# M-Igashi/mp3rgain

Measured on AMD Instinct MI355X. Metric: stereo PCM samples/s through IIR+RMS+histogram, higher is better.
Workload: dtype f64

## Files before the change

mp3rgain_amd/csrc/rg_capi.hip:

```cpp
#include <atomic>
#include <chrono>
#include <hip/hip_runtime.h>

#include <dlfcn.h>
#include <math.h>
#include <stdarg.h>
#include <stdio.h>
#include <string.h>

#include <string>
#include <vector>

#include "rg_ctx.h"

extern "C" {
hipError_t rg_launch_k1_halo(const RgTrackDev *, uint32_t, uint32_t, const RgCoefDev *, uint32_t *,
                             unsigned long long *, unsigned long long *, hipStream_t);
hipError_t rg_launch_track_results(const uint32_t *, const unsigned long long *, const RgTrackDev *,
                                   const unsigned long long *, rg_track_result *, uint32_t, hipStream_t);
hipError_t rg_launch_album_merge(const uint32_t *, const unsigned long long *, uint32_t, uint32_t *, double *,
                                 hipStream_t);
hipError_t rg_launch_album_result(const uint32_t *, const double *, rg_album_result *, hipStream_t);
hipError_t rg_launch_album_reduce_gathered(const uint32_t *, uint32_t, uint32_t *, double *, hipStream_t);
hipError_t rg_launch_peak_all(const void *, uint64_t, uint32_t, unsigned long long *, hipStream_t);
hipError_t rg_launch_synth_fill(float *, uint64_t, uint32_t, uint32_t, uint64_t, uint64_t, hipStream_t);
}

namespace {
thread_local std::string g_create_error;
}

int rg_set_err(rg_ctx *c, int code, const char *fmt, ...) {
    char buf[512];
    va_list ap;
    va_start(ap, fmt);
    vsnprintf(buf, sizeof buf, fmt, ap);
    va_end(ap);
    if (c) c->err = buf; else g_create_error = buf;
    return code;
}

int rg_rate_index(uint32_t sr) {
    for (int i = 0; i < RG_NUM_RATES; ++i)
        if (RG_RATE_TABLE[i].sample_rate == sr) return i;
    return -1;
}

int rg_bind_device(rg_ctx *c) {
    RG_HIP(c, hipSetDevice(c->device));
    return RG_OK;
}

namespace {

int32_t round_to_i32(double v) {
    double r = round(v);
    if (r != r) return 0;
    if (r >= 2147483647.0) return INT32_MAX;
    if (r <= -2147483648.0) return INT32_MIN;
    return (int32_t)r;
}

int drain_timing(rg_ctx *c) {
    for (int k = 0; k < RG_MAX_SLOTS; ++k) {
        RgSlot &S = c->slots[k];
        for (size_t i = 0; i < S.ev_used; ++i) {
            float ms = 0.f;
            RG_HIP(c, hipEventElapsedTime(&ms, S.ev_pool[i].first, S.ev_pool[i].second));
            c->timing_sum_ms += ms;
            c->timing_count += 1;
// ... 151 lines not shown
        else S.stream = c->slots[k % RG_SLOT_STREAMS].stream;
        if (e == hipSuccess) e = hipEventCreateWithFlags(&S.staging_done, hipEventDisableTiming);
        if (e == hipSuccess) e = hipEventCreateWithFlags(&S.batch_done, hipEventDisableTiming);
        if (e == hipSuccess) e = hipEventCreateWithFlags(&S.album_done, hipEventDisableTiming);
        if (e == hipSuccess) e = S.d_album_hist.reserve(RG_HISTOGRAM_SIZE + 2);
        if (e == hipSuccess) S.d_album_peak.p = reinterpret_cast<double *>(S.d_album_hist.p + RG_HISTOGRAM_SIZE);
        if (e == hipSuccess) e = S.d_album_result.reserve(1);
        if (e == hipSuccess) e = S.h_album_result.reserve(1);
    }
    if (e != hipSuccess) {
        rg_set_err(nullptr, RG_ERR_DEVICE, "stream / buffer creation: %s", hipGetErrorString(e));
        rg_destroy(c);
        return nullptr;
    }

    std::vector<RgCoefDev> coefs(RG_NUM_RATES);
    for (int i = 0; i < RG_NUM_RATES; ++i) {
        rg_design_rate(RG_RATE_TABLE[i], &c->design[i]);
        memcpy(coefs[i].ya, RG_RATE_TABLE[i].yule_a, sizeof coefs[i].ya);
        memcpy(coefs[i].yb, RG_RATE_TABLE[i].yule_b, sizeof coefs[i].yb);
        memcpy(coefs[i].ba, RG_RATE_TABLE[i].butter_a, sizeof coefs[i].ba);
        memcpy(coefs[i].bb, RG_RATE_TABLE[i].butter_b, sizeof coefs[i].bb);
    }
    if ((e = c->d_coefs.reserve(RG_NUM_RATES)) != hipSuccess ||
        (e = hipMemcpy(c->d_coefs.p, coefs.data(), sizeof(RgCoefDev) * RG_NUM_RATES, hipMemcpyHostToDevice)) !=
            hipSuccess) {
        rg_set_err(nullptr, RG_ERR_DEVICE, "context allocation: %s", hipGetErrorString(e));
        rg_destroy(c);
        return nullptr;
    }
    check_hw_queues(c);
    return c;
}

extern "C" void rg_destroy(rg_ctx *c) {
    if (!c) return;
    (void)hipSetDevice(c->device);
    (void)sync_all(c);
    (void)rg_comm_destroy(c);
    for (int k = 0; k < RG_MAX_SLOTS; ++k) {
        RgSlot &S = c->slots[k];
        for (auto &p : S.ev_pool) {
            (void)hipEventDestroy(p.first);
            (void)hipEventDestroy(p.second);
        }
        S.d_desc.release();
        S.h_desc.release();
        S.d_tm_rec.release();
        S.d_tm_win.release();
        S.d_hist.release();
        S.d_nonfinite.release();
        S.d_imprecise.release();
        S.d_k1_bad.release();
        S.d_results.release();
        S.h_results.release();
        S.d_album_hist.release();
        S.d_album_peak.p = nullptr;
        S.d_album_result.release();
        S.d_gather.release();
        S.h_album_result.release();
        if (S.staging_done) (void)hipEventDestroy(S.staging_done);
        if (S.batch_done) (void)hipEventDestroy(S.batch_done);
        if (S.album_done) (void)hipEventDestroy(S.album_done);
        if (S.stream && k < RG_SLOT_STREAMS) (void)hipStreamDestroy(S.stream);
    }
    if (c->user_ev) (void)hipEventDestroy(c->user_ev);
    c->d_coefs.release();
    c->d_peak_bits.release();
    c->d_arena.release();
    c->d_wav.release();
    c->d_flac_blob.release();
    c->d_flac_work.release();
    c->h_flac_stage.release();
    c->d_flac_md5.release();
    c->d_mp3_crc.release();
    c->d_rip.release();
    c->d_stats.release();
    c->d_spectrum.release();
    c->d_dr.release();
    c->d_stereo.release();
    c->d_clicks.release();
    c->d_flacenc.release();
    c->d_flacenc_out.release();
    c->d_flacenc_verify.release();
    c->d_ancestry.release();
    c->d_fprint.release();
    c->d_fp_codes.release();
    c->d_tempo.release();
    c->d_tp_onsets.release();
    c->d_key.release();
    c->d_key_decim.release();
    c->d_key_rows.release();
    c->d_rs.release();
    c->d_rs_y.release();
    c->h_mp3_crc.release();
    if (c->file_pool && c->file_pool_free) c->file_pool_free(c->file_pool);
    c->file_pool = nullptr;
    c->d_mp3_tab.release();
    c->d_mp3_is.release();
    c->d_mp3_units.release();
    c->d_mp3_tracks.release();
    c->d_mp3_huff.release();
    c->d_mp3_recs.release();
    c->d_mp3_main.release();
    if (c->mp3_pipe && c->mp3_pipe_free) c->mp3_pipe_free(c->mp3_pipe);
    c->mp3_pipe = nullptr;
// ... 716 lines not shown
```

mp3rgain_amd/csrc/rg_ctx.h:

```cpp
#pragma once

#include <hip/hip_runtime.h>

#include <map>
#include <string>
#include <vector>

#include "rg_design.h"
#include "rg_device.h"
#include "rg_tm.h"

template <typename T>
struct DevBuf {
    T *p = nullptr;
    size_t cap = 0;
    hipError_t reserve(size_t n) {
        if (n <= cap) return hipSuccess;
        if (p) (void)hipFree(p);
        p = nullptr;
        cap = 0;
        size_t want = n + n / 4 + 16;
        hipError_t e = hipMalloc((void **)&p, want * sizeof(T));
        if (e == hipSuccess) cap = want;
        return e;
// ... 5 lines not shown
    }
};

template <typename T>
struct PinnedBuf {
    T *p = nullptr;
    size_t cap = 0;
    hipError_t reserve(size_t n) {
        if (n <= cap) return hipSuccess;
        if (p) (void)hipHostFree(p);
        p = nullptr;
        cap = 0;
        size_t want = n + n / 4 + 16;
        hipError_t e = hipHostMalloc((void **)&p, want * sizeof(T), hipHostMallocDefault);
        if (e == hipSuccess) cap = want;
        return e;
    }
    void release() {
        if (p) (void)hipHostFree(p);
        p = nullptr;
        cap = 0;
    }
};

struct RgTmDeviceTables {
    RgTmDesign design;
    double *d_blob = nullptr;
    RgTmGeom geom{};
    RgTmFixTables fix{};
};

enum { RG_TUNE_TM_SEGMENT = 1, RG_TUNE_TM_TARGET_LANES = 2, RG_TUNE_PIPELINE_SLOTS = 3, RG_TUNE_TM_WINDOWS = 4, RG_TUNE_INGEST_CHUNK_KIB = 5,
       RG_TUNE_GPU_MP3_DECODE = 6, RG_TUNE_LOADER_THREADS = 7, RG_TUNE_ALBUM_PARTS = 10, RG_TUNE_PARTS_MIN_BPU = 11,
       RG_TUNE_STAGE_BYTES = 12, RG_TUNE_GROUP_BYTES = 13, RG_TUNE_GPU_FLAC_DECODE = 14 };

#define RG_MAX_SLOTS 8
#define RG_SLOT_STREAMS 4
#define RG_DEFAULT_SLOTS 8

struct RgSlot {
    hipStream_t stream = nullptr;
    hipEvent_t staging_done = nullptr;
    hipEvent_t batch_done = nullptr;
    hipEvent_t album_done = nullptr;
    bool album_pending = false;
    bool staging_pending = false;
    DevBuf<unsigned char> d_desc;
    PinnedBuf<unsigned char> h_desc;
    std::vector<unsigned char> desc_shadow;
    DevBuf<double> d_tm_rec;
    DevBuf<double> d_tm_win;
    DevBuf<uint32_t> d_hist;
    DevBuf<unsigned long long> d_k1_bad;
    DevBuf<uint32_t> d_imprecise;
    DevBuf<uint32_t> d_nonfinite;
    unsigned long long *peak_ptr = nullptr;
    DevBuf<rg_track_result> d_results;
    PinnedBuf<rg_track_result> h_results;
    DevBuf<uint32_t> d_album_hist;
    DevBuf<double> d_album_peak;
    DevBuf<rg_album_result> d_album_result;
    DevBuf<uint32_t> d_gather;
    PinnedBuf<rg_album_result> h_album_result;
    size_t n_enqueued = 0;
    int enq_album = 0;
    const void *enq_base = nullptr;
    size_t enq_bytes = 0;
    bool album_ready = false;
    std::vector<std::pair<hipEvent_t, hipEvent_t>> ev_pool;
    size_t ev_used = 0;
};

struct rg_ctx {
    int device = -1;
    std::string err;
    int kernel_variant = 0;
    uint32_t tune_tm_segment = 0;
    uint32_t tune_tm_windows = 0;
    uint64_t tune_tm_target_lanes = 0;
    int n_slots = RG_DEFAULT_SLOTS;

    RgSlot slots[RG_MAX_SLOTS];
    int cur = 0;
    hipStream_t user_stream = nullptr;
    bool user_attached = false;
    hipEvent_t user_ev = nullptr;
    bool user_dirty = false;
    RgSlot &slot() { return slots[cur]; }
    hipStream_t album_stream() { return user_attached ? user_stream : slots[cur].stream; }
    hipStream_t file_stream() { return album_stream(); }

    RgRateDesign design[RG_NUM_RATES];
    DevBuf<RgCoefDev> d_coefs;
    std::map<uint32_t, RgTmDeviceTables *> tm_tables;

    std::map<uint64_t, std::pair<uint32_t, uint32_t>> tm_choice;

    std::vector<RgTrackDev> h_tracks, h_k1_tracks;
    std::vector<RgTmTrack> h_tm_tracks;

    DevBuf<unsigned long long> d_peak_bits;
    DevBuf<unsigned char> d_mp3_tab;
    DevBuf<int16_t> d_mp3_is;
    DevBuf<unsigned char> d_mp3_units;
    DevBuf<unsigned char> d_mp3_tracks;
    DevBuf<unsigned char> d_mp3_huff;
    DevBuf<unsigned char> d_mp3_recs;
    DevBuf<unsigned char> d_mp3_main;
    bool mp3_tab_ready = false;
    DevBuf<unsigned char> d_mp3_stage[2];
    hipStream_t mp3_copy_stream = nullptr;
    hipEvent_t mp3_set_free[2] = {nullptr, nullptr};
    bool mp3_set_used[2] = {false, false};
    DevBuf<uint32_t> d_mp3_results;
    DevBuf<uint32_t> d_mp3_tiles;
    DevBuf<unsigned char> d_mp3_recs_set[2];
    DevBuf<uint32_t> d_mp3_tiles_set[2];
    DevBuf<uint32_t> d_mp3_perm_set[2];
    DevBuf<uint32_t> d_mp3_sortw_set[2];
    PinnedBuf<uint32_t> h_mp3_results;
    hipEvent_t enqueue_wait_ev = nullptr;
    hipStream_t enqueue_stream = nullptr;
    PinnedBuf<uint32_t> h_mp3_part_counts;
    PinnedBuf<rg_track_result> h_part_results;
    hipEvent_t *mp3_bench_ev = nullptr;
    void *mp3_pipe = nullptr;
    void (*mp3_pipe_free)(void *) = nullptr;
    void *file_pool = nullptr;
    std::vector<std::string> file_errors;
    void (*file_pool_free)(void *) = nullptr;
    int gpu_mp3_decode = 3;
    int gpu_flac_decode = 1;
    DevBuf<unsigned char> d_flac_blob;
    DevBuf<unsigned char> d_flac_work;
    PinnedBuf<unsigned char> h_flac_stage;
    DevBuf<unsigned char> d_flac_md5;
    DevBuf<unsigned char> d_mp3_crc;
    PinnedBuf<unsigned char> h_mp3_crc;
    DevBuf<unsigned char> d_rip;
    DevBuf<unsigned char> d_stats;
    DevBuf<unsigned char> d_spectrum;
    DevBuf<unsigned char> d_dr;
    DevBuf<unsigned char> d_stereo;
    DevBuf<unsigned char> d_clicks;
    DevBuf<unsigned char> d_flacenc;
    DevBuf<unsigned char> d_flacenc_out;
// ... 90 lines not shown
```

mp3rgain_amd/csrc/rg_device.h:

```cpp
#pragma once

#include <stdint.h>

#include "../../include/mp3rgain_amd.h"
#include "../../include/rg_coeffs.h"

#define RG_MAX_TAPS 11

struct RgCoefDev {
    double ya[11];
    double yb[11];
    double ba[3];
    double bb[3];
};

struct RgTrackDev {
    const void *ch0;
    const void *ch1;
    uint64_t frames;
    uint32_t window;
    uint32_t n_windows;
    uint32_t seg_windows;
    uint32_t n_segments;
    uint32_t halo;
    uint32_t coef_idx;
    uint32_t format;
    uint32_t item_base;
    uint32_t sample_rate;
    uint32_t file_type;
    uint32_t track_index;
    uint32_t pad_;
};

#define RG_ONE_MINUS_PERCENTILE (1.0 - 0.95)
```

mp3rgain_amd/csrc/rg_enqueue.hip:

```cpp
#include <stdlib.h>
#include <string.h>

#include <math.h>

#include <algorithm>

#include "rg_ctx.h"

extern "C" {
hipError_t rg_launch_k1_halo(const RgTrackDev *, uint32_t, uint32_t, const RgCoefDev *, uint32_t *,
                             unsigned long long *, unsigned long long *, hipStream_t);
hipError_t rg_launch_track_results(const uint32_t *, const unsigned long long *, const RgTrackDev *,
                                   const unsigned long long *, rg_track_result *, uint32_t, hipStream_t);
hipError_t rg_launch_album_merge(const uint32_t *, const unsigned long long *, uint32_t, uint32_t *, double *,
                                 hipStream_t);
hipError_t rg_launch_tm_main(int fmt, int nch, const RgTmCoef *, const RgTmGeom *, const RgTmTrack *, uint32_t, uint32_t,
                             double *, uint32_t, double *, uint32_t, uint32_t *, uint32_t *, uint64_t, hipStream_t);
hipError_t rg_launch_tm_fix(int nch, const RgTmGeom *, const RgTmFixTables *, const RgTmTrack *, uint32_t, uint32_t,
                            const double *, uint32_t, const double *, uint32_t, uint32_t *, uint32_t *, uint32_t *,
                            unsigned long long *, uint32_t *, rg_track_result *, hipStream_t);
}

namespace {

const uint32_t kMinSegment = 96;

struct TmGroup {
    int rate_idx, fmt, nch;
    std::vector<uint32_t> ids;
    uint64_t frames = 0;
};

int validate(rg_ctx *c, const rg_track_desc *tracks, size_t n, size_t pcm_bytes) {
    for (size_t t = 0; t < n; ++t) {
        const rg_track_desc &d = tracks[t];
        if (rg_rate_index(d.sample_rate) < 0)
            return rg_set_err(c, RG_ERR_UNSUPPORTED_RATE,
                              "Unsupported sample rate: %u Hz. Supported rates: 96000, 88200, 64000, 48000, 44100, "
                              "32000, 24000, 22050, 16000, 12000, 11025, 8000",
                              d.sample_rate);
        if (d.channels == 0) return rg_set_err(c, RG_ERR_INVALID_ARG, "track %zu: channels == 0", t);
        if (d.format > RG_FMT_S32_PLANAR) return rg_set_err(c, RG_ERR_INVALID_ARG, "track %zu: unknown format %u", t, d.format);
        const size_t bps = rg_bytes_per_sample(d.format);
        if (d.offset_bytes % bps) return rg_set_err(c, RG_ERR_INVALID_ARG, "track %zu: offset not sample-aligned", t);
        const uint64_t need = d.offset_bytes + (uint64_t)d.channels * d.frames * bps;
        if (need > pcm_bytes)
            return rg_set_err(c, RG_ERR_INVALID_ARG, "track %zu: extends past the PCM arena (%llu > %zu)", t,
                              (unsigned long long)need, pcm_bytes);
        const uint32_t W = rg_window_samples(d.sample_rate);
        if ((d.frames + W - 1) / W > 0x7FFFFFFFull) return rg_set_err(c, RG_ERR_INVALID_ARG, "track %zu: too long", t);
    }
    return RG_OK;
}

void fill_common(rg_ctx *c, const rg_track_desc &d, const unsigned char *d_base, uint32_t track_index, RgTrackDev &o) {
    const int ri = rg_rate_index(d.sample_rate);
    const size_t bps = rg_bytes_per_sample(d.format);
    memset(&o, 0, sizeof o);
    o.ch0 = d_base + d.offset_bytes;
    o.ch1 = d.channels >= 2 ? d_base + d.offset_bytes + d.frames * bps : nullptr;
    o.frames = d.frames;
    o.window = rg_window_samples(d.sample_rate);
    o.n_windows = (uint32_t)((d.frames + o.window - 1) / o.window);
    o.coef_idx = (uint32_t)ri;
    o.format = d.format;
    o.sample_rate = d.sample_rate;
    o.file_type = RG_FILE_MP3;
    o.track_index = track_index;
    (void)c;
}

int finish_k1_list(rg_ctx *c, RgTrackDev *list, size_t n, uint32_t *total_items) {
    uint64_t total_windows = 0;
    for (size_t t = 0; t < n; ++t) total_windows += list[t].n_windows;
    uint32_t seg_windows = 1;
    if (total_windows > (1u << 18)) {
        uint64_t s = total_windows >> 17;
        seg_windows = (uint32_t)(s > 16 ? 16 : s);
    }
    uint64_t items = 0;
    for (size_t t = 0; t < n; ++t) {
        RgTrackDev &o = list[t];
        if (t > 0 && list[t - 1].coef_idx != o.coef_idx) items = (items + 63) & ~(uint64_t)63;
        if (c->design[o.coef_idx].stable) {
            o.seg_windows = seg_windows;
            o.halo = c->design[o.coef_idx].halo_frames;
        } else {
            o.seg_windows = o.n_windows ? o.n_windows : 1;
            o.halo = 0xFFFFFFFFu;
        }
        o.n_segments = (o.n_windows + o.seg_windows - 1) / o.seg_windows;
        o.item_base = (uint32_t)items;
        items += o.n_segments;
        if (items > 0x7FFFFFFFull) return rg_set_err(c, RG_ERR_INVALID_ARG, "batch too large");
    }
    *total_items = (uint32_t)items;
    return RG_OK;
}

int get_tm_tables(rg_ctx *c, int rate_idx, uint32_t L, RgTmDeviceTables **out, uint32_t m = 1) {
    const uint32_t key = ((uint32_t)rate_idx << 24) | (m << 16) | L;
    auto it = c->tm_tables.find(key);
    if (it != c->tm_tables.end()) {
        *out = it->second;
        return it->second->design.ok ? RG_OK : RG_ERR_INVALID_ARG;
    }
    RgTmDeviceTables *tb = new RgTmDeviceTables();
    rg_tm_design(RG_RATE_TABLE[rate_idx], L, &tb->design, m);
    c->tm_tables[key] = tb;
    *out = tb;
    const RgTmDesign &D = tb->design;
    if (!D.ok) return RG_ERR_INVALID_ARG;
    const size_t nT = D.T.size(), nG = D.Gp.size(), nY = D.PhiY.size(), nB = D.PhiB.size();
    const size_t nL = (size_t)D.H10 * 12 + (size_t)(D.L - D.H10) * 2;
    const size_t nST = D.ST.size();
    const size_t total = nT + nG + nY + nB + 24 + 12 + 100 + 12 + 8 + nL + 2 + nST;
    std::vector<double> blob(total, 0.0);
    size_t o = 0;
    const size_t oT = o; memcpy(&blob[o], D.T.data(), nT * 8); o += nT;
    const size_t oG = o; memcpy(&blob[o], D.Gp.data(), nG * 8); o += nG;
    const size_t oY = o; if (nY) memcpy(&blob[o], D.PhiY.data(), nY * 8); o += nY;
    const size_t oB = o; if (nB) memcpy(&blob[o], D.PhiB.data(), nB * 8); o += nB;
    const size_t oX = o; memcpy(&blob[o], &D.Xs[0][0], 24 * 8); o += 24;
    const size_t oS = o; memcpy(&blob[o], D.sigma0, 12 * 8); o += 12;
    memcpy(&blob[o], D.Wf, 100 * 8); o += 100;
    if (nST) memcpy(&blob[o], &D.ST[(size_t)(D.L - 1) * 12], 12 * 8);
    o += 12;
    o = (o + 1) & ~(size_t)1;
    const size_t oL = o;
    for (uint32_t n = 0; n < D.H10; ++n)
        for (int j = 0; j < 12; ++j) blob[o++] = D.T[(size_t)n * 12 + j];
    for (uint32_t n = D.H10; n < D.L; ++n) { blob[o++] = D.T[(size_t)n * 12 + 10]; blob[o++] = D.T[(size_t)n * 12 + 11]; }
    o = (o + 1) & ~(size_t)1;
    const size_t oST = o;
    if (nST) memcpy(&blob[o], D.ST.data(), nST * 8);
    o += nST;
    RG_HIP(c, hipMalloc((void **)&tb->d_blob, total * 8));
    RG_HIP(c, hipMemcpy(tb->d_blob, blob.data(), total * 8, hipMemcpyHostToDevice));
    RgTmGeom &g = tb->geom;
    g.L = D.L;
    g.W = D.W;
    g.k = D.W / D.L;
    g.H10 = D.H10;
    g.rounds = D.rounds;
    g.rounds_fast = D.rounds_fast;
    g.warm = 1u << D.rounds;
    g.fix_windows = (RG_TM_BLOCK - g.warm) / g.k;
    g.block = rg_tm_choose_block(D.L, D.H10, m);
    g.m = m;
// ... 173 lines not shown
    if (S.album_pending) {
        RG_HIP(c, hipStreamWaitEvent(s, S.album_done, 0));
        S.album_pending = false;
    }

    if (S.staging_pending) {
        RG_HIP(c, hipEventSynchronize(S.staging_done));
        S.staging_pending = false;
    }

    c->h_tracks.resize(n ? n : 1);
    c->h_k1_tracks.resize(n ? n : 1);
    c->h_tm_tracks.resize(n ? n : 1);
    const size_t acc_words = n * (size_t)(RG_HISTOGRAM_SIZE + 3);
    RG_HIP(c, S.d_hist.reserve(acc_words));
    S.peak_ptr = reinterpret_cast<unsigned long long *>(S.d_hist.p + n * (size_t)RG_HISTOGRAM_SIZE);
    uint32_t *const done_ptr = S.d_hist.p + n * (size_t)(RG_HISTOGRAM_SIZE + 2);
    RG_HIP(c, S.d_results.reserve(n));
    RG_HIP(c, S.h_results.reserve(n));
    if (n > S.d_nonfinite.cap) {
        RG_HIP(c, S.d_nonfinite.reserve(n));
        RG_HIP(c, hipMemsetAsync(S.d_nonfinite.p, 0, S.d_nonfinite.cap * sizeof(uint32_t), s));
    }
    if (n > S.d_imprecise.cap) {
        RG_HIP(c, S.d_imprecise.reserve(n));
        RG_HIP(c, hipMemsetAsync(S.d_imprecise.p, 0, S.d_imprecise.cap * sizeof(uint32_t), s));
    }

    const unsigned char *base = (const unsigned char *)d_pcm_base;
    const bool use_tm = c->kernel_variant != 1;

    std::vector<TmGroup> groups;
    size_t n_k1 = 0;
    for (size_t t = 0; t < n; ++t) {
        fill_common(c, tracks[t], base, (uint32_t)t, c->h_tracks[t]);
        const int ri = rg_rate_index(tracks[t].sample_rate);
        const bool tm_rate = !(c->force_exact.size() == n && c->force_exact[t]);
        if (use_tm && tm_rate && c->design[ri].stable) {
            const int nch = tracks[t].channels >= 2 ? 2 : 1;
            TmGroup *g = nullptr;
            for (auto &q : groups)
                if (q.rate_idx == ri && q.fmt == (int)tracks[t].format && q.nch == nch) { g = &q; break; }
            if (!g) {
                groups.push_back(TmGroup{ri, (int)tracks[t].format, nch, {}, 0});
                g = &groups.back();
            }
            g->ids.push_back((uint32_t)t);
            g->frames += tracks[t].frames;
        } else {
            c->h_k1_tracks[n_k1++] = c->h_tracks[t];
        }
    }
    uint32_t k1_items = 0;
    rc = finish_k1_list(c, c->h_k1_tracks.data(), n_k1, &k1_items);
    if (rc != RG_OK) return rc;

    struct GroupLaunch {
        RgTmDeviceTables *tb;
        RgTmCoef K;
        size_t list_off, list_n;
        uint32_t main_grid, fix_grid, total_recs, total_windows;
        int fmt, nch;
    };
    std::vector<GroupLaunch> launches;
    size_t tm_off = 0;
    size_t max_rec_doubles = 0, max_win_doubles = 0;
    for (const TmGroup &g : groups) {
        GroupLaunch gl{};
        rc = choose_tm_tables(c, g, tracks, &gl.tb);
        if (rc != RG_OK) return rc;
        const RgTmGeom &geo = gl.tb->geom;
        const rg_rate_coeffs &rcf = RG_RATE_TABLE[g.rate_idx];
        const double scale = g.fmt == RG_FMT_F32_PLANAR ? 32768.0 : (g.fmt == RG_FMT_S16_PLANAR ? 1.0 : 32768.0 / 2147483648.0);
        const RgTmDesign &des = gl.tb->design;
        for (int i = 0; i < 11; ++i) {
            gl.K.b[i] = (des.servo ? (double)((long double)des.g * (long double)rcf.yule_b[i]) : rcf.yule_b[i]) * scale;
            gl.K.a[i] = rcf.yule_a[i];
        }
        for (int i = 0; i < 3; ++i) { gl.K.bb[i] = rcf.butter_b[i]; gl.K.ba[i] = rcf.butter_a[i]; }
        gl.K.c0 = 1e-10;
        gl.K.alpha = des.alpha;
        gl.K.beta = des.beta;
        gl.K.aff_lin = geo.aff_lin;
        gl.K.aff_n = geo.aff_n;
        gl.fmt = g.fmt;
        gl.nch = g.nch;
        gl.list_off = tm_off;
        gl.list_n = g.ids.size();
        uint64_t recs = 0, mb = 0, fb = 0, wins = 0;
        const uint64_t seg_stride = (uint64_t)geo.L * geo.m;
        const uint32_t NB = geo.fix_windows * geo.k;
        const uint32_t geom_block = geo.block;
        for (uint32_t id : g.ids) {
            const RgTrackDev &cd = c->h_tracks[id];
            RgTmTrack &o = c->h_tm_tracks[tm_off++];
            o.ch0 = cd.ch0;
            o.ch1 = cd.ch1;
            o.frames = cd.frames;
            o.nseg = (uint32_t)((cd.frames + seg_stride - 1) / seg_stride);
            o.n_windows = cd.n_windows;
            o.rec_base = (uint32_t)recs;
            o.lane_base = (uint32_t)mb;
            o.fix_block_base = (uint32_t)fb;
            o.track_index = id;
            o.fix_blocks = (o.nseg + NB - 1) / NB;
            o.sample_rate = cd.sample_rate;
            o.file_type = cd.file_type;
// ... 27 lines not shown
    S.enq_base = d_pcm_base;
    S.enq_bytes = pcm_bytes;
    S.album_ready = false;
    const RgTrackDev *d_tracks = nullptr, *d_k1_tracks = nullptr;
    const RgTmTrack *d_tm_tracks = nullptr;
    if (n) {
        const size_t o_all = 0;
        const size_t o_k1 = (o_all + n * sizeof(RgTrackDev) + 15) & ~(size_t)15;
        const size_t o_tm = (o_k1 + n_k1 * sizeof(RgTrackDev) + 15) & ~(size_t)15;
        const size_t blob_bytes = o_tm + tm_off * sizeof(RgTmTrack);
        const size_t old_desc_cap = S.d_desc.cap;
        RG_HIP(c, S.d_desc.reserve(blob_bytes));
        RG_HIP(c, S.h_desc.reserve(blob_bytes));
        if (S.d_desc.cap != old_desc_cap) S.desc_shadow.clear();
        std::vector<unsigned char> blob(blob_bytes, 0);
        memcpy(&blob[o_all], c->h_tracks.data(), n * sizeof(RgTrackDev));
        if (n_k1) memcpy(&blob[o_k1], c->h_k1_tracks.data(), n_k1 * sizeof(RgTrackDev));
        if (tm_off) memcpy(&blob[o_tm], c->h_tm_tracks.data(), tm_off * sizeof(RgTmTrack));
        if (blob != S.desc_shadow) {
            memcpy(S.h_desc.p, blob.data(), blob_bytes);
            RG_HIP(c, hipMemcpyAsync(S.d_desc.p, S.h_desc.p, blob_bytes, hipMemcpyHostToDevice, s));
            RG_HIP(c, hipEventRecord(S.staging_done, s));
            S.staging_pending = true;
            S.desc_shadow.swap(blob);
        }
        d_tracks = reinterpret_cast<const RgTrackDev *>(S.d_desc.p + o_all);
        (void)d_tracks;
        d_k1_tracks = reinterpret_cast<const RgTrackDev *>(S.d_desc.p + o_k1);
        d_tm_tracks = reinterpret_cast<const RgTmTrack *>(S.d_desc.p + o_tm);
        bool cleared = false;
        bool any_main = false;
        for (const GroupLaunch &gl : launches) any_main = any_main || gl.main_grid != 0;
        if (!any_main) {
            RG_HIP(c, hipMemsetAsync(S.d_hist.p, 0, acc_words * sizeof(uint32_t), s));
            cleared = true;
        }

        for (const GroupLaunch &gl : launches) {
            hipEvent_t e1;
            rc = timing_begin(c, &e1);
            if (rc != RG_OK) return rc;
            RG_HIP(c, rg_launch_tm_main(gl.fmt, gl.nch, &gl.K, &gl.tb->geom, d_tm_tracks + gl.list_off,
                                        (uint32_t)gl.list_n, gl.main_grid, S.d_tm_rec.p, gl.total_recs, S.d_tm_win.p,
                                        gl.total_windows, S.d_nonfinite.p, cleared ? nullptr : S.d_hist.p, (uint64_t)acc_words, s));
            if (gl.main_grid != 0) cleared = true;
            if (e1) RG_HIP(c, hipEventRecord(e1, s));
            RG_HIP(c, rg_launch_tm_fix(gl.nch, &gl.tb->geom, &gl.tb->fix, d_tm_tracks + gl.list_off,
                                       (uint32_t)gl.list_n, gl.fix_grid, S.d_tm_rec.p, gl.total_recs, S.d_tm_win.p,
                                       gl.total_windows, S.d_nonfinite.p, S.d_imprecise.p, S.d_hist.p, S.peak_ptr, done_ptr, S.d_results.p, s));
        }
        if (n_k1) {
            RG_HIP(c, S.d_k1_bad.reserve(n));
            RG_HIP(c, hipMemsetAsync(S.d_k1_bad.p, 0xFF, n * sizeof(unsigned long long), s));
            hipEvent_t e1;
            rc = timing_begin(c, &e1);
            if (rc != RG_OK) return rc;
            RG_HIP(c, rg_launch_k1_halo(d_k1_tracks, (uint32_t)n_k1, k1_items, c->d_coefs.p, S.d_hist.p,
                                        S.peak_ptr, S.d_k1_bad.p, s));
            if (e1) RG_HIP(c, hipEventRecord(e1, s));
        }
        RG_HIP(c, rg_launch_track_results(S.d_hist.p, S.peak_ptr, d_k1_tracks, S.d_k1_bad.p, S.d_results.p, (uint32_t)n_k1, s));
    }
    if (album) {
        RG_HIP(c, rg_launch_album_merge(S.d_hist.p, S.peak_ptr, (uint32_t)n, S.d_album_hist.p,
                                        S.d_album_peak.p, s));
        S.album_ready = true;
        if (c->user_attached) {
            RG_HIP(c, hipEventRecord(S.batch_done, s));
            RG_HIP(c, hipStreamWaitEvent(c->user_stream, S.batch_done, 0));
        }
    }
    return RG_OK;
}
```

mp3rgain_amd/csrc/rg_k1_halo.hip:

```cpp
#include <hip/hip_runtime.h>
#include <limits.h>

#include <type_traits>

#include "rg_device.h"
#include "rg_device_inl.h"

#define RG_K1_ELEVEN(f)                                                                                       \
    do {                                                                                                      \
        f(std::integral_constant<int, 0>{}); f(std::integral_constant<int, 1>{}); f(std::integral_constant<int, 2>{});   \
        f(std::integral_constant<int, 3>{});                                                                             \
        __builtin_amdgcn_sched_barrier(0);       \
        f(std::integral_constant<int, 4>{}); f(std::integral_constant<int, 5>{}); f(std::integral_constant<int, 6>{});   \
        f(std::integral_constant<int, 7>{});                                                                             \
        __builtin_amdgcn_sched_barrier(0);                                                                              \
        f(std::integral_constant<int, 8>{}); f(std::integral_constant<int, 9>{}); f(std::integral_constant<int, 10>{}); \
    } while (0)

#define RG_K1_TWELVE(f)                                                                                       \
    do {                                                                                                      \
        f(std::integral_constant<int, 0>{}); f(std::integral_constant<int, 1>{}); f(std::integral_constant<int, 2>{});   \
        f(std::integral_constant<int, 3>{});                                                                             \
        __builtin_amdgcn_sched_barrier(0);                                                                              \
        f(std::integral_constant<int, 4>{}); f(std::integral_constant<int, 5>{}); f(std::integral_constant<int, 6>{});   \
// ... 21 lines not shown
    for (int i = 10; i >= 1; --i) { f.yx[i] = f.yx[i - 1]; f.yy[i] = f.yy[i - 1]; }
    f.yx[0] = s;
    double acc = 0.0;
#pragma unroll
    for (int i = 1; i < 11; ++i) {
        double t = c.yb[i] * f.yx[i] - c.ya[i] * f.yy[i];
        acc = acc + t;
    }
    const double y = (1e-10 + c.yb[0] * f.yx[0]) + acc;
    f.yy[0] = y;

    f.bx[2] = f.bx[1]; f.bx[1] = f.bx[0];
    f.by[2] = f.by[1]; f.by[1] = f.by[0];
    f.bx[0] = y;
    double acc2 = 0.0;
#pragma unroll
    for (int i = 1; i < 3; ++i) {
        double t = c.bb[i] * f.bx[i] - c.ba[i] * f.by[i];
        acc2 = acc2 + t;
    }
    const double z = (1e-10 + c.bb[0] * f.bx[0]) + acc2;
    f.by[0] = z;
    return z;
}

template <int K>
__device__ __forceinline__ double df1_process_rot(Df1State &f, const RgCoefDev &c, double s) {
    constexpr int P0 = (11 - K) % 12;
    f.yx[P0] = s;
    double acc = 0.0;
#pragma unroll
    for (int i = 1; i < 11; ++i) {
        const int p = (i - K - 1 + 24) % 12;
        double t = c.yb[i] * f.yx[p] - c.ya[i] * f.yy[p];
        acc = acc + t;
    }
    const double y = (1e-10 + c.yb[0] * f.yx[P0]) + acc;
    f.yy[P0] = y;

    f.bx[2] = f.bx[1]; f.bx[1] = f.bx[0];
    f.by[2] = f.by[1]; f.by[1] = f.by[0];
    f.bx[0] = y;
    double acc2 = 0.0;
#pragma unroll
    for (int i = 1; i < 3; ++i) {
        double t = c.bb[i] * f.bx[i] - c.ba[i] * f.by[i];
        acc2 = acc2 + t;
    }
    const double z = (1e-10 + c.bb[0] * f.bx[0]) + acc2;
    f.by[0] = z;
    return z;
}

__device__ __forceinline__ double load_input(const void *base, uint64_t i, uint32_t fmt, double &mag) {
    if (fmt == RG_FMT_F32_PLANAR) {
        const double xn = (double)((const float *)base)[i];
        mag = fabs(xn);
        return xn * 32768.0;
    } else if (fmt == RG_FMT_S16_PLANAR) {
        const double v = (double)((const int16_t *)base)[i];
        mag = fabs(v / 32768.0);
        return v;
    } else {
        const double v = (double)((const int32_t *)base)[i] * (32768.0 / 2147483648.0);
        mag = fabs(v / 32768.0);
        return v;
    }
}

__device__ __forceinline__ double cvt_input(uint32_t w, uint32_t fmt, double &mag) {
    if (fmt == RG_FMT_F32_PLANAR) {
        const double xn = (double)__uint_as_float(w);
        mag = fabs(xn);
        return xn * 32768.0;
    } else if (fmt == RG_FMT_S16_PLANAR) {
        const double v = (double)(int32_t)w;
        mag = fabs(v / 32768.0);
        return v;
    } else {
        const double v = (double)(int32_t)w * (32768.0 / 2147483648.0);
        mag = fabs(v / 32768.0);
        return v;
    }
}

typedef uint32_t __attribute__((ext_vector_type(4), aligned(4))) k1_u32x4u;
typedef short __attribute__((ext_vector_type(4), aligned(2))) k1_s16x4u;

__device__ __forceinline__ uint4 load_piece(const void *base, uint64_t i, uint32_t fmt) {
    if (fmt == RG_FMT_S16_PLANAR) {
        const k1_s16x4u v = *(const k1_s16x4u *)((const int16_t *)base + i);
        return make_uint4((uint32_t)(int32_t)v.x, (uint32_t)(int32_t)v.y, (uint32_t)(int32_t)v.z, (uint32_t)(int32_t)v.w);
    }
    const k1_u32x4u v = *(const k1_u32x4u *)((const uint32_t *)base + i);
    return make_uint4(v.x, v.y, v.z, v.w);
}

}

__global__ void __launch_bounds__(256) rg_k1_first_nonfinite_kernel(const RgTrackDev *__restrict__ tracks,
                                                                    unsigned long long *__restrict__ first_bad, uint32_t n_tracks) {
  for (uint32_t t = blockIdx.y; t < n_tracks; t += gridDim.y) {
    const RgTrackDev tr = tracks[t];
    if (tr.format != RG_FMT_F32_PLANAR) continue;
    const uint64_t stride = (uint64_t)gridDim.x * blockDim.x;
    unsigned long long best = ~0ull;
    for (uint64_t i = (uint64_t)blockIdx.x * blockDim.x + threadIdx.x; i < tr.frames; i += stride) {
        const float a = ((const float *)tr.ch0)[i];
        const float b = tr.ch1 ? ((const float *)tr.ch1)[i] : 0.0f;
        if (!(fabsf(a) <= 3.402823466e38f) || !(fabsf(b) <= 3.402823466e38f)) { best = i; break; }
    }
    if (best != ~0ull) atomicMin(&first_bad[tr.track_index], best);
  }
}

__global__ void __launch_bounds__(256) rg_k1_halo_kernel(const RgTrackDev *__restrict__ tracks, uint32_t n_tracks,
                                                         uint32_t total_items, const RgCoefDev *__restrict__ coefs,
                                                         uint32_t *__restrict__ hist,
                                                         unsigned long long *__restrict__ peak_bits,
                                                         const unsigned long long *__restrict__ first_bad) {
    const uint32_t g = blockIdx.x * blockDim.x + threadIdx.x;
    if (g >= total_items) return;

    uint32_t lo = 0, hi = n_tracks - 1;
    while (lo < hi) {
        const uint32_t mid = (lo + hi + 1) >> 1;
        if (tracks[mid].item_base <= g) lo = mid; else hi = mid - 1;
    }
    const uint32_t t = lo;
    const RgTrackDev tr = tracks[t];
    const uint32_t seg = g - tr.item_base;
    if (seg >= tr.n_segments) return;
    const RgCoefDev c = coefs[__builtin_amdgcn_readfirstlane(tr.coef_idx)];

    const uint64_t W = tr.window;
    const uint64_t first = (uint64_t)seg * tr.seg_windows * W;
    uint64_t last = first + (uint64_t)tr.seg_windows * W;
    if (last > tr.frames) last = tr.frames;
    const uint64_t warm = (tr.halo != 0xFFFFFFFFu && first > tr.halo) ? first - tr.halo : 0;
    const bool stereo = tr.ch1 != nullptr;
    const uint32_t fmt = tr.format;

    Df1State fl, fr;
    df1_reset(fl);
    df1_reset(fr);
    double mag;

    double peak = 0.0, lsum = 0.0, rsum = 0.0;
    uint32_t n = 0;
    uint32_t *const h = hist + (size_t)tr.track_index * RG_HISTOGRAM_SIZE;
    const uint64_t bad_from = first_bad[tr.track_index];
    const double qnan = __longlong_as_double(0x7FF8000000000000ll);
    auto frame = [&](const uint64_t i, const double xl, const double ml, const double xr, const double mr, auto rot) {
        constexpr int ROT = decltype(rot)::value;
        double lf, rf = 0.0;
        if constexpr (ROT >= 0) lf = df1_process_rot<ROT>(fl, c, xl);
        else lf = df1_process(fl, c, xl);
        if (stereo) {
            if constexpr (ROT >= 0) rf = df1_process_rot<ROT>(fr, c, xr);
            else rf = df1_process(fr, c, xr);
        }
        if (i < first) return;
        if (ml > peak) peak = ml;
        if (stereo) {
            if (mr > peak) peak = mr;
            lsum += lf * lf;
            rsum += rf * rf;
        } else {
            const double sq = lf * lf;
            lsum += sq;
            rsum += sq;
        }
        if (++n >= W) {
            if (i + 1 - n > bad_from) lsum = qnan;
            const int idx = rg_window_bin(lsum, rsum, n);
            if (idx >= 0) atomicAdd(&h[idx], 1u);
            lsum = 0.0; rsum = 0.0; n = 0;
        }
    };
    {
        uint64_t i = warm;
        uint4 pl[3], pr[3];
        if (i + 12 <= last) {
#pragma unroll
            for (int p = 0; p < 3; ++p) {
                pl[p] = load_piece(tr.ch0, i + 4u * p, fmt);
                if (stereo) pr[p] = load_piece(tr.ch1, i + 4u * p, fmt);
            }
        }
        for (; i + 12 <= last; i += 12) {
            const bool more = i + 24 <= last;
            auto four = [&](auto piece) {
                constexpr int P = decltype(piece)::value;
                const uint32_t wl[4] = {pl[P].x, pl[P].y, pl[P].z, pl[P].w};
                const uint32_t wr[4] = {pr[P].x, pr[P].y, pr[P].z, pr[P].w};
                if (more) {
                    pl[P] = load_piece(tr.ch0, i + 12u + 4u * P, fmt);
                    if (stereo) pr[P] = load_piece(tr.ch1, i + 12u + 4u * P, fmt);
                }
                auto step = [&](auto k) {
                    constexpr int K = decltype(k)::value;
                    double ml, mr = 0.0, xr = 0.0;
                    const double xl = cvt_input(wl[K & 3], fmt, ml);
                    if (stereo) xr = cvt_input(wr[K & 3], fmt, mr);
                    frame(i + K, xl, ml, xr, mr, k);
                };
                step(std::integral_constant<int, 4 * P>{});
                step(std::integral_constant<int, 4 * P + 1>{});
                step(std::integral_constant<int, 4 * P + 2>{});
                step(std::integral_constant<int, 4 * P + 3>{});
                __builtin_amdgcn_sched_barrier(0);
            };
            four(std::integral_constant<int, 0>{});
            four(std::integral_constant<int, 1>{});
            four(std::integral_constant<int, 2>{});
        }
        for (; i < last; ++i) {
            double ml, mr = 0.0, xr = 0.0;
            const double xl = load_input(tr.ch0, i, fmt, ml);
            if (stereo) xr = load_input(tr.ch1, i, fmt, mr);
            frame(i, xl, ml, xr, mr, std::integral_constant<int, -1>{});
        }
    }
    (void)mag;
    if (n > 0) {
        if (last - n > bad_from) lsum = qnan;
        const int idx = rg_window_bin(lsum, rsum, n);
        if (idx >= 0) atomicAdd(&h[idx], 1u);
    }
    atomicMax(&peak_bits[tr.track_index], (unsigned long long)__double_as_longlong(peak));
}

extern "C" hipError_t rg_launch_k1_halo(const RgTrackDev *d_tracks, uint32_t n_tracks, uint32_t total_items,
                                        const RgCoefDev *d_coefs, uint32_t *d_hist,
                                        unsigned long long *d_peak_bits, unsigned long long *d_first_bad ,
                                        hipStream_t stream) {
    if (total_items == 0) return hipSuccess;
    hipLaunchKernelGGL(rg_k1_first_nonfinite_kernel, dim3(512, n_tracks < 65535u ? n_tracks : 65535u), dim3(256), 0, stream, d_tracks,
                       d_first_bad, n_tracks);
    const uint32_t block = 64;
    const uint32_t grid = (total_items + block - 1) / block;
    hipLaunchKernelGGL(rg_k1_halo_kernel, dim3(grid), dim3(block), 0, stream, d_tracks, n_tracks, total_items,
                       d_coefs, d_hist, d_peak_bits, d_first_bad);
    return hipGetLastError();
}
```

Before: 452.5 billion.

## Split stereo channels across lanes, fuse nonfinite scan, size segments to residency

Each stereo track now gets two lanes, one per channel, and the pair combines window sums with a shuffle. This halves per-lane serial IIR work and doubles parallelism. The separate pre-pass that scanned every sample for non-finite values is removed. Detection is folded into the main kernel and a per-window bin record, with a small fix-up kernel that re-bins windows after the first bad sample. Segment length is now picked from the device's resident lane count, minimising waves times segment length, replacing a fixed heuristic. In exchange it adds a per-window bin buffer write, extra atomics and a second launch.

```diff
diff --git a/mp3rgain_amd/csrc/rg_capi.hip b/mp3rgain_amd/csrc/rg_capi.hip
--- a/mp3rgain_amd/csrc/rg_capi.hip
+++ b/mp3rgain_amd/csrc/rg_capi.hip
@@ -15,7 +15,7 @@
 
 extern "C" {
 hipError_t rg_launch_k1_halo(const RgTrackDev *, uint32_t, uint32_t, const RgCoefDev *, uint32_t *,
-                             unsigned long long *, unsigned long long *, hipStream_t);
+                             unsigned long long *, unsigned long long *, int32_t *, hipStream_t);
 hipError_t rg_launch_track_results(const uint32_t *, const unsigned long long *, const RgTrackDev *,
                                    const unsigned long long *, rg_track_result *, uint32_t, hipStream_t);
 hipError_t rg_launch_album_merge(const uint32_t *, const unsigned long long *, uint32_t, uint32_t *, double *,
@@ -273,6 +273,7 @@
         S.d_nonfinite.release();
         S.d_imprecise.release();
         S.d_k1_bad.release();
+        S.d_k1_bins.release();
         S.d_results.release();
         S.h_results.release();
         S.d_album_hist.release();
diff --git a/mp3rgain_amd/csrc/rg_ctx.h b/mp3rgain_amd/csrc/rg_ctx.h
--- a/mp3rgain_amd/csrc/rg_ctx.h
+++ b/mp3rgain_amd/csrc/rg_ctx.h
@@ -81,6 +81,7 @@
     DevBuf<double> d_tm_win;
     DevBuf<uint32_t> d_hist;
     DevBuf<unsigned long long> d_k1_bad;
+    DevBuf<int32_t> d_k1_bins;
     DevBuf<uint32_t> d_imprecise;
     DevBuf<uint32_t> d_nonfinite;
     unsigned long long *peak_ptr = nullptr;
@@ -121,6 +122,7 @@
 
     RgRateDesign design[RG_NUM_RATES];
     DevBuf<RgCoefDev> d_coefs;
+    uint32_t k1_resident_lanes = 0;
     std::map<uint32_t, RgTmDeviceTables *> tm_tables;
 
     std::map<uint64_t, std::pair<uint32_t, uint32_t>> tm_choice;
diff --git a/mp3rgain_amd/csrc/rg_device.h b/mp3rgain_amd/csrc/rg_device.h
--- a/mp3rgain_amd/csrc/rg_device.h
+++ b/mp3rgain_amd/csrc/rg_device.h
@@ -29,7 +29,7 @@
     uint32_t sample_rate;
     uint32_t file_type;
     uint32_t track_index;
-    uint32_t pad_;
+    uint32_t win_base;
 };
 
 #define RG_ONE_MINUS_PERCENTILE (1.0 - 0.95)
diff --git a/mp3rgain_amd/csrc/rg_enqueue.hip b/mp3rgain_amd/csrc/rg_enqueue.hip
--- a/mp3rgain_amd/csrc/rg_enqueue.hip
+++ b/mp3rgain_amd/csrc/rg_enqueue.hip
@@ -9,7 +9,8 @@
 
 extern "C" {
 hipError_t rg_launch_k1_halo(const RgTrackDev *, uint32_t, uint32_t, const RgCoefDev *, uint32_t *,
-                             unsigned long long *, unsigned long long *, hipStream_t);
+                             unsigned long long *, unsigned long long *, int32_t *, hipStream_t);
+hipError_t rg_k1_resident_lanes(int device, uint32_t *lanes);
 hipError_t rg_launch_track_results(const uint32_t *, const unsigned long long *, const RgTrackDev *,
                                    const unsigned long long *, rg_track_result *, uint32_t, hipStream_t);
 hipError_t rg_launch_album_merge(const uint32_t *, const unsigned long long *, uint32_t, uint32_t *, double *,
@@ -70,31 +71,91 @@
     (void)c;
 }
 
-int finish_k1_list(rg_ctx *c, RgTrackDev *list, size_t n, uint32_t *total_items) {
-    uint64_t total_windows = 0;
-    for (size_t t = 0; t < n; ++t) total_windows += list[t].n_windows;
-    uint32_t seg_windows = 1;
-    if (total_windows > (1u << 18)) {
-        uint64_t s = total_windows >> 17;
-        seg_windows = (uint32_t)(s > 16 ? 16 : s);
-    }
-    uint64_t items = 0;
+}
+
+extern "C" int rg_k1_split(const uint32_t *n_windows, const uint32_t *window, const uint32_t *halo, const uint32_t *rate_row,
+                           const uint32_t *channels, size_t n, uint32_t resident_lanes, uint32_t *seg_windows,
+                           uint32_t *n_segments, uint32_t *lane_base, uint64_t *total_lanes) {
+    uint64_t lanes_at_one = 0, frames_max = 0, halo_max = 0;
+    for (size_t t = 0; t < n; ++t)
+        if (halo[t] != 0xFFFFFFFFu) {
+            lanes_at_one += (uint64_t)n_windows[t] * (channels[t] >= 2 ? 2 : 1);
+            frames_max = std::max<uint64_t>(frames_max, window[t]);
+            halo_max = std::max<uint64_t>(halo_max, halo[t]);
+        }
+    auto lay_out = [&](uint32_t s, bool write) {
+        uint64_t lanes = 0;
+        for (size_t t = 0; t < n; ++t) {
+            if (t > 0 && rate_row[t - 1] != rate_row[t]) lanes = (lanes + 63) & ~(uint64_t)63;
+            const uint32_t nch = channels[t] >= 2 ? 2 : 1;
+            if (nch == 2) lanes = (lanes + 1) & ~(uint64_t)1;
+            const uint32_t sw = halo[t] != 0xFFFFFFFFu ? s : (n_windows[t] ? n_windows[t] : 1);
+            const uint32_t ns = (uint32_t)(((uint64_t)n_windows[t] + sw - 1) / sw);
+            if (write) {
+                seg_windows[t] = sw;
+                n_segments[t] = ns;
+                lane_base[t] = (uint32_t)lanes;
+            }
+            lanes += (uint64_t)ns * nch;
+        }
+        return lanes;
+    };
+    uint32_t s_best = 1;
+    const uint64_t R = resident_lanes;
+    if (R && lanes_at_one > 2 * R) {
+        double best = 0.0;
+        for (uint64_t k = 1; k <= 4; ++k) {
+            uint64_t s = (lanes_at_one + k * R - 1) / (k * R);
+            uint64_t lanes = lay_out((uint32_t)s, false);
+            for (int tries = 0; lanes > k * R && tries < 64 && s < 0x7FFFFFFFull; ++tries) lanes = lay_out((uint32_t)++s, false);
+            if (lanes > k * R) continue;
+            const double cost = (double)((lanes + R - 1) / R) * (double)(s * frames_max + halo_max);
+            if (best == 0.0 || cost < best) { best = cost; s_best = (uint32_t)s; }
+        }
+    }
+    const uint64_t lanes = lay_out(s_best, true);
+    *total_lanes = lanes;
+    return lanes > 0x7FFFFFFFull ? -1 : 0;
+}
+
+namespace {
+
+int finish_k1_list(rg_ctx *c, RgTrackDev *list, size_t n, uint32_t *total_items, size_t *total_bins) {
+    *total_items = 0;
+    *total_bins = 0;
+    if (n == 0) return RG_OK;
+    bool any_split = false;
+    std::vector<uint32_t> v(8 * n);
+    uint32_t *const nw = v.data(), *const win = nw + n, *const halo = win + n, *const row = halo + n, *const nch = row + n,
+                    *const sw = nch + n, *const ns = sw + n, *const base = ns + n;
+    for (size_t t = 0; t < n; ++t) {
+        const RgTrackDev &o = list[t];
+        nw[t] = o.n_windows;
+        win[t] = o.window;
+        row[t] = o.coef_idx;
+        nch[t] = o.ch1 ? 2 : 1;
+        halo[t] = c->design[o.coef_idx].stable ? c->design[o.coef_idx].halo_frames : 0xFFFFFFFFu;
+        any_split = any_split || halo[t] != 0xFFFFFFFFu;
+    }
+    if (any_split && !c->k1_resident_lanes) RG_HIP(c, rg_k1_resident_lanes(c->device, &c->k1_resident_lanes));
+    uint64_t items = 0, bins = 0;
+    if (rg_k1_split(nw, win, halo, row, nch, n, c->k1_resident_lanes, sw, ns, base, &items) != 0)
+        return rg_set_err(c, RG_ERR_INVALID_ARG, "batch too large");
     for (size_t t = 0; t < n; ++t) {
         RgTrackDev &o = list[t];
-        if (t > 0 && list[t - 1].coef_idx != o.coef_idx) items = (items + 63) & ~(uint64_t)63;
-        if (c->design[o.coef_idx].stable) {
-            o.seg_windows = seg_windows;
-            o.halo = c->design[o.coef_idx].halo_frames;
-        } else {
-            o.seg_windows = o.n_windows ? o.n_windows : 1;
-            o.halo = 0xFFFFFFFFu;
-        }
-        o.n_segments = (o.n_windows + o.seg_windows - 1) / o.seg_windows;
-        o.item_base = (uint32_t)items;
-        items += o.n_segments;
-        if (items > 0x7FFFFFFFull) return rg_set_err(c, RG_ERR_INVALID_ARG, "batch too large");
+        o.seg_windows = sw[t];
+        o.n_segments = ns[t];
+        o.halo = halo[t];
+        o.item_base = base[t];
+        o.win_base = 0;
+        if (o.format == RG_FMT_F32_PLANAR && o.halo != 0xFFFFFFFFu) {
+            o.win_base = (uint32_t)bins;
+            bins += o.n_windows;
+            if (bins > 0x7FFFFFFFull) return rg_set_err(c, RG_ERR_INVALID_ARG, "batch too large");
+        }
     }
     *total_items = (uint32_t)items;
+    *total_bins = (size_t)bins;
     return RG_OK;
 }
 
@@ -374,7 +435,8 @@
         }
     }
     uint32_t k1_items = 0;
-    rc = finish_k1_list(c, c->h_k1_tracks.data(), n_k1, &k1_items);
+    size_t k1_bins = 0;
+    rc = finish_k1_list(c, c->h_k1_tracks.data(), n_k1, &k1_items, &k1_bins);
     if (rc != RG_OK) return rc;
 
     struct GroupLaunch {
@@ -508,11 +570,12 @@
         if (n_k1) {
             RG_HIP(c, S.d_k1_bad.reserve(n));
             RG_HIP(c, hipMemsetAsync(S.d_k1_bad.p, 0xFF, n * sizeof(unsigned long long), s));
+            RG_HIP(c, S.d_k1_bins.reserve(k1_bins ? k1_bins : 1));
             hipEvent_t e1;
             rc = timing_begin(c, &e1);
             if (rc != RG_OK) return rc;
             RG_HIP(c, rg_launch_k1_halo(d_k1_tracks, (uint32_t)n_k1, k1_items, c->d_coefs.p, S.d_hist.p,
-                                        S.peak_ptr, S.d_k1_bad.p, s));
+                                        S.peak_ptr, S.d_k1_bad.p, S.d_k1_bins.p, s));
             if (e1) RG_HIP(c, hipEventRecord(e1, s));
         }
         RG_HIP(c, rg_launch_track_results(S.d_hist.p, S.peak_ptr, d_k1_tracks, S.d_k1_bad.p, S.d_results.p, (uint32_t)n_k1, s));
diff --git a/mp3rgain_amd/csrc/rg_k1_halo.hip b/mp3rgain_amd/csrc/rg_k1_halo.hip
--- a/mp3rgain_amd/csrc/rg_k1_halo.hip
+++ b/mp3rgain_amd/csrc/rg_k1_halo.hip
@@ -97,9 +97,11 @@
     return z;
 }
 
-__device__ __forceinline__ double load_input(const void *base, uint64_t i, uint32_t fmt, double &mag) {
+__device__ __forceinline__ double load_input(const void *base, uint64_t i, uint32_t fmt, double &mag, bool &bad) {
     if (fmt == RG_FMT_F32_PLANAR) {
-        const double xn = (double)((const float *)base)[i];
+        const float x = ((const float *)base)[i];
+        bad |= !(fabsf(x) <= 3.402823466e38f);
+        const double xn = (double)x;
         mag = fabs(xn);
         return xn * 32768.0;
     } else if (fmt == RG_FMT_S16_PLANAR) {
@@ -113,9 +115,11 @@
     }
 }
 
-__device__ __forceinline__ double cvt_input(uint32_t w, uint32_t fmt, double &mag) {
+__device__ __forceinline__ double cvt_input(uint32_t w, uint32_t fmt, double &mag, bool &bad) {
     if (fmt == RG_FMT_F32_PLANAR) {
-        const double xn = (double)__uint_as_float(w);
+        const float x = __uint_as_float(w);
+        bad |= !(fabsf(x) <= 3.402823466e38f);
+        const double xn = (double)x;
         mag = fabs(xn);
         return xn * 32768.0;
     } else if (fmt == RG_FMT_S16_PLANAR) {
@@ -143,29 +147,14 @@
 
 }
 
-__global__ void __launch_bounds__(256) rg_k1_first_nonfinite_kernel(const RgTrackDev *__restrict__ tracks,
-                                                                    unsigned long long *__restrict__ first_bad, uint32_t n_tracks) {
-  for (uint32_t t = blockIdx.y; t < n_tracks; t += gridDim.y) {
-    const RgTrackDev tr = tracks[t];
-    if (tr.format != RG_FMT_F32_PLANAR) continue;
-    const uint64_t stride = (uint64_t)gridDim.x * blockDim.x;
-    unsigned long long best = ~0ull;
-    for (uint64_t i = (uint64_t)blockIdx.x * blockDim.x + threadIdx.x; i < tr.frames; i += stride) {
-        const float a = ((const float *)tr.ch0)[i];
-        const float b = tr.ch1 ? ((const float *)tr.ch1)[i] : 0.0f;
-        if (!(fabsf(a) <= 3.402823466e38f) || !(fabsf(b) <= 3.402823466e38f)) { best = i; break; }
-    }
-    if (best != ~0ull) atomicMin(&first_bad[tr.track_index], best);
-  }
-}
-
 __global__ void __launch_bounds__(256) rg_k1_halo_kernel(const RgTrackDev *__restrict__ tracks, uint32_t n_tracks,
-                                                         uint32_t total_items, const RgCoefDev *__restrict__ coefs,
+                                                         uint32_t total_lanes, const RgCoefDev *__restrict__ coefs,
                                                          uint32_t *__restrict__ hist,
                                                          unsigned long long *__restrict__ peak_bits,
-                                                         const unsigned long long *__restrict__ first_bad) {
+                                                         unsigned long long *__restrict__ first_bad,
+                                                         int32_t *__restrict__ win_bin) {
     const uint32_t g = blockIdx.x * blockDim.x + threadIdx.x;
-    if (g >= total_items) return;
+    if (g >= total_lanes) return;
 
     uint32_t lo = 0, hi = n_tracks - 1;
     while (lo < hi) {
@@ -174,7 +163,10 @@
     }
     const uint32_t t = lo;
     const RgTrackDev tr = tracks[t];
-    const uint32_t seg = g - tr.item_base;
+    const bool stereo = tr.ch1 != nullptr;
+    const uint32_t local = g - tr.item_base;
+    const uint32_t seg = stereo ? local >> 1 : local;
+    const uint32_t ch = stereo ? local & 1u : 0u;
     if (seg >= tr.n_segments) return;
     const RgCoefDev c = coefs[__builtin_amdgcn_readfirstlane(tr.coef_idx)];
 
@@ -183,72 +175,59 @@
     uint64_t last = first + (uint64_t)tr.seg_windows * W;
     if (last > tr.frames) last = tr.frames;
     const uint64_t warm = (tr.halo != 0xFFFFFFFFu && first > tr.halo) ? first - tr.halo : 0;
-    const bool stereo = tr.ch1 != nullptr;
     const uint32_t fmt = tr.format;
-
-    Df1State fl, fr;
-    df1_reset(fl);
-    df1_reset(fr);
-    double mag;
-
-    double peak = 0.0, lsum = 0.0, rsum = 0.0;
+    const void *const pcm = ch ? tr.ch1 : tr.ch0;
+
+    Df1State f;
+    df1_reset(f);
+
+    double peak = 0.0, sum = 0.0;
     uint32_t n = 0;
     uint32_t *const h = hist + (size_t)tr.track_index * RG_HISTOGRAM_SIZE;
-    const uint64_t bad_from = first_bad[tr.track_index];
-    const double qnan = __longlong_as_double(0x7FF8000000000000ll);
-    auto frame = [&](const uint64_t i, const double xl, const double ml, const double xr, const double mr, auto rot) {
-        constexpr int ROT = decltype(rot)::value;
-        double lf, rf = 0.0;
-        if constexpr (ROT >= 0) lf = df1_process_rot<ROT>(fl, c, xl);
-        else lf = df1_process(fl, c, xl);
-        if (stereo) {
-            if constexpr (ROT >= 0) rf = df1_process_rot<ROT>(fr, c, xr);
-            else rf = df1_process(fr, c, xr);
-        }
-        if (i < first) return;
-        if (ml > peak) peak = ml;
-        if (stereo) {
-            if (mr > peak) peak = mr;
-            lsum += lf * lf;
-            rsum += rf * rf;
-        } else {
-            const double sq = lf * lf;
-            lsum += sq;
-            rsum += sq;
-        }
-        if (++n >= W) {
-            if (i + 1 - n > bad_from) lsum = qnan;
+    unsigned long long *const bad_from = first_bad + tr.track_index;
+    int32_t *wb = (fmt == RG_FMT_F32_PLANAR && tr.halo != 0xFFFFFFFFu && ch == 0)
+                      ? win_bin + tr.win_base + (size_t)seg * tr.seg_windows : nullptr;
+    bool bad = false;
+    auto window_end = [&](const uint64_t start) {
+        if (bad) { atomicMin(bad_from, (unsigned long long)start); bad = false; }
+        const double other = __shfl_xor(sum, 1, 64);
+        const double lsum = (stereo && ch) ? other : sum;
+        const double rsum = (stereo && !ch) ? other : sum;
+        if (ch == 0) {
             const int idx = rg_window_bin(lsum, rsum, n);
             if (idx >= 0) atomicAdd(&h[idx], 1u);
-            lsum = 0.0; rsum = 0.0; n = 0;
-        }
+            if (wb) *wb++ = idx;
+        }
+        sum = 0.0; n = 0;
+    };
+    auto frame = [&](const uint64_t i, const double x, const double m, auto rot) {
+        constexpr int ROT = decltype(rot)::value;
+        double y;
+        if constexpr (ROT >= 0) y = df1_process_rot<ROT>(f, c, x);
+        else y = df1_process(f, c, x);
+        if (i < first) return;
+        if (m > peak) peak = m;
+        sum += y * y;
+        if (++n >= W) window_end(i + 1 - n);
     };
     {
         uint64_t i = warm;
-        uint4 pl[3], pr[3];
+        uint4 pc[3];
         if (i + 12 <= last) {
 #pragma unroll
-            for (int p = 0; p < 3; ++p) {
-                pl[p] = load_piece(tr.ch0, i + 4u * p, fmt);
-                if (stereo) pr[p] = load_piece(tr.ch1, i + 4u * p, fmt);
-            }
+            for (int p = 0; p < 3; ++p) pc[p] = load_piece(pcm, i + 4u * p, fmt);
         }
         for (; i + 12 <= last; i += 12) {
             const bool more = i + 24 <= last;
             auto four = [&](auto piece) {
                 constexpr int P = decltype(piece)::value;
-                const uint32_t wl[4] = {pl[P].x, pl[P].y, pl[P].z, pl[P].w};
-                const uint32_t wr[4] = {pr[P].x, pr[P].y, pr[P].z, pr[P].w};
-                if (more) {
-                    pl[P] = load_piece(tr.ch0, i + 12u + 4u * P, fmt);
-                    if (stereo) pr[P] = load_piece(tr.ch1, i + 12u + 4u * P, fmt);
-                }
+                const uint32_t w[4] = {pc[P].x, pc[P].y, pc[P].z, pc[P].w};
+                if (more) pc[P] = load_piece(pcm, i + 12u + 4u * P, fmt);
                 auto step = [&](auto k) {
                     constexpr int K = decltype(k)::value;
-                    double ml, mr = 0.0, xr = 0.0;
-                    const double xl = cvt_input(wl[K & 3], fmt, ml);
-                    if (stereo) xr = cvt_input(wr[K & 3], fmt, mr);
-                    frame(i + K, xl, ml, xr, mr, k);
+                    double m;
+                    const double x = cvt_input(w[K & 3], fmt, m, bad);
+                    frame(i + K, x, m, k);
                 };
                 step(std::integral_constant<int, 4 * P>{});
                 step(std::integral_constant<int, 4 * P + 1>{});
@@ -261,31 +240,56 @@
             four(std::integral_constant<int, 2>{});
         }
         for (; i < last; ++i) {
-            double ml, mr = 0.0, xr = 0.0;
-            const double xl = load_input(tr.ch0, i, fmt, ml);
-            if (stereo) xr = load_input(tr.ch1, i, fmt, mr);
-            frame(i, xl, ml, xr, mr, std::integral_constant<int, -1>{});
-        }
-    }
-    (void)mag;
-    if (n > 0) {
-        if (last - n > bad_from) lsum = qnan;
-        const int idx = rg_window_bin(lsum, rsum, n);
-        if (idx >= 0) atomicAdd(&h[idx], 1u);
-    }
+            double m;
+            const double x = load_input(pcm, i, fmt, m, bad);
+            frame(i, x, m, std::integral_constant<int, -1>{});
+        }
+    }
+    if (n > 0) window_end(last - n);
     atomicMax(&peak_bits[tr.track_index], (unsigned long long)__double_as_longlong(peak));
 }
 
-extern "C" hipError_t rg_launch_k1_halo(const RgTrackDev *d_tracks, uint32_t n_tracks, uint32_t total_items,
+__global__ void __launch_bounds__(256) rg_k1_nonfinite_fix_kernel(const RgTrackDev *__restrict__ tracks, uint32_t n_tracks,
+                                                                  uint32_t *__restrict__ hist,
+                                                                  const unsigned long long *__restrict__ first_bad,
+                                                                  const int32_t *__restrict__ win_bin) {
+    for (uint32_t t = blockIdx.x; t < n_tracks; t += gridDim.x) {
+        const RgTrackDev tr = tracks[t];
+        if (tr.format != RG_FMT_F32_PLANAR || tr.halo == 0xFFFFFFFFu || tr.n_segments == 0) continue;
+        const unsigned long long bad_from = first_bad[tr.track_index];
+        if (bad_from == ~0ull) continue;
+        uint32_t *const h = hist + (size_t)tr.track_index * RG_HISTOGRAM_SIZE;
+        const int nan_bin = rg_window_bin(__longlong_as_double(0x7FF8000000000000ll), 0.0, 1u);
+        for (uint64_t w = bad_from / tr.window + 1 + threadIdx.x; w < tr.n_windows; w += blockDim.x) {
+            const int32_t b = win_bin[tr.win_base + w];
+            if (b >= 0) atomicSub(&h[b], 1u);
+            if (nan_bin >= 0) atomicAdd(&h[nan_bin], 1u);
+        }
+    }
+}
+
+extern "C" hipError_t rg_k1_resident_lanes(int device, uint32_t *lanes) {
+    int blocks = 0, cus = 0;
+    hipError_t e = hipOccupancyMaxActiveBlocksPerMultiprocessor(&blocks, rg_k1_halo_kernel, 64, 0);
+    if (e != hipSuccess) return e;
+    e = hipDeviceGetAttribute(&cus, hipDeviceAttributeMultiprocessorCount, device);
+    if (e != hipSuccess) return e;
+    if (blocks <= 0 || cus <= 0) return hipErrorInvalidValue;
+    *lanes = (uint32_t)blocks * (uint32_t)cus * 64u;
+    return hipSuccess;
+}
+
+extern "C" hipError_t rg_launch_k1_halo(const RgTrackDev *d_tracks, uint32_t n_tracks, uint32_t total_lanes,
                                         const RgCoefDev *d_coefs, uint32_t *d_hist,
                                         unsigned long long *d_peak_bits, unsigned long long *d_first_bad ,
+                                        int32_t *d_win_bin ,
                                         hipStream_t stream) {
-    if (total_items == 0) return hipSuccess;
-    hipLaunchKernelGGL(rg_k1_first_nonfinite_kernel, dim3(512, n_tracks < 65535u ? n_tracks : 65535u), dim3(256), 0, stream, d_tracks,
-                       d_first_bad, n_tracks);
+    if (total_lanes == 0) return hipSuccess;
     const uint32_t block = 64;
-    const uint32_t grid = (total_items + block - 1) / block;
-    hipLaunchKernelGGL(rg_k1_halo_kernel, dim3(grid), dim3(block), 0, stream, d_tracks, n_tracks, total_items,
-                       d_coefs, d_hist, d_peak_bits, d_first_bad);
+    const uint32_t grid = (total_lanes + block - 1) / block;
+    hipLaunchKernelGGL(rg_k1_halo_kernel, dim3(grid), dim3(block), 0, stream, d_tracks, n_tracks, total_lanes,
+                       d_coefs, d_hist, d_peak_bits, d_first_bad, d_win_bin);
+    hipLaunchKernelGGL(rg_k1_nonfinite_fix_kernel, dim3(n_tracks < 1024u ? n_tracks : 1024u), dim3(256), 0, stream, d_tracks,
+                       n_tracks, d_hist, d_first_bad, d_win_bin);
     return hipGetLastError();
 }
```

Result: no change. 452.9 billion (median of 5 runs) (+0.1%).
